# alanqrwang/nwhead

Hardware: AMD Instinct MI355X
Metric: query-predictions/sec (higher is better)
Workload: dtype f32; 1 GPU; K3 predict('full'): B=256 queries/step vs bank N=50000 d=512 C=200, bank sharded 1-way, 26 query batches coalesced per launch; B=256, N_support=50000, d=512, C=200, parallelism=support-shard x1

## Files before the change

### include/nwhead_hip.h

```cpp
#ifndef NWHEAD_HIP_H
#define NWHEAD_HIP_H

#include <stddef.h>
#include <stdint.h>

#ifdef __cplusplus
extern "C" {
#endif

#define NW_ABI_VERSION 2

typedef enum {
    NW_SCORE_EUCLIDEAN = 0,
    NW_SCORE_HYPERSPHERE = 1,
    NW_SCORE_COSINE = 2,
    NW_SCORE_DOT = 3,
    NW_SCORE_CLIP = 4
} nw_score_kind;

typedef enum {
    NW_OK = 0,
    NW_ERR_INVALID_ARG = -1,
    NW_ERR_UNSUPPORTED = -2,
    NW_ERR_WORKSPACE = -3,
    NW_ERR_LAUNCH = -4,
    NW_ERR_NO_DEVICE = -5
} nw_status;

int nw_abi_version(void);
const char *nw_status_string(int status);
int nw_device_check(void);

int nw_scores_f32(const float *q, const float *s, float *scores,
                  int64_t B, int64_t N, int64_t d,
                  int kind, const float *logit_scale_dev, int sup_batched, void *stream);

int nw_row_norm2_f32(const float *x, float *n2, int64_t rows, int64_t d, void *stream);

int nw_split_rows_f16x2(const float *x, float *out_split, float *row_scale, float *row_norm2,
                        int64_t rows, int64_t d, void *stream);

int nw_pack_rows_f16(const float *x, uint16_t *out_rows, float *row_scale, float *row_norm2,
                     int64_t rows, int64_t d, void *stream);

typedef struct nw_fwd_opts {
    uint32_t struct_size;
    int32_t persistent_wgs;
    int32_t force_split;
    int32_t operand_form;
    const void *tables;
    size_t tables_bytes;
    const int64_t *tables_sy;
    int64_t tables_N;
} nw_fwd_opts;

size_t nw_fwd_workspace_bytes(int64_t B, int64_t N, int64_t d, int64_t C);
int nw_fwd_f32(const float *q, const float *s, const int64_t *sy, const float *s_norm2,
               const float *s_split, const float *s_scale,
               float *out, float *scores_out, float *lse_out, float *weights_out,
               void *workspace, size_t workspace_bytes,
               int64_t B, int64_t N, int64_t d, int64_t C,
               int kind, const float *logit_scale_dev,
               int sup_batched, int labels_batched, const nw_fwd_opts *opts, void *stream);

int nw_fwd_partial_f32(const float *q, const float *s, const int64_t *sy, const float *s_norm2,
                       const float *s_split, const float *s_scale,
                       float *m, float *den, float *num,
                       void *workspace, size_t workspace_bytes,
                       int64_t B, int64_t N, int64_t d, int64_t C,
                       int kind, const float *logit_scale_dev, const nw_fwd_opts *opts, void *stream);
int nw_merge_finalize_f32(const float *m, const float *den, const float *num, float *out,
                          int64_t G, int64_t B, int64_t C,
                          int64_t stride_m, int64_t stride_den, int64_t stride_num,
                          const int64_t *class_lo, int64_t C_local, void *stream);

size_t nw_bank_tables_bytes(int64_t N);
int nw_bank_tables_build(const int64_t *sy, int64_t N, int64_t C, void *tables, size_t tables_bytes, void *stream);


size_t nw_bwd_workspace_bytes(int64_t B, int64_t N, int64_t d, int64_t C, int kind, int sup_batched);
int nw_bwd_f32(const float *q, const float *s, const int64_t *sy,
               const float *scores, const float *lse, const float *out, const float *gout,
               float *gq, float *gs, float *glogit_scale,
               void *workspace, size_t workspace_bytes,
               int64_t B, int64_t N, int64_t d, int64_t C,
               int kind, const float *logit_scale_dev,
               int sup_batched, int labels_batched, void *stream);
int nw_bwd_uses_split(int64_t B, int64_t N, int64_t d, int64_t C, int sup_batched);
int nw_bwd_bank_f32(const float *q, const float *s, const float *s_norm2, const float *s_split,
                    const float *s_scale, const int64_t *sy,
                    const float *scores, const float *lse, const float *out, const float *gout,
                    float *gq, float *gs, float *glogit_scale,
                    void *workspace, size_t workspace_bytes,
                    int64_t B, int64_t N, int64_t d, int64_t C,
                    int kind, const float *logit_scale_dev,
                    int sup_batched, int labels_batched, void *stream);


int nw_support_influence_f32(const float *probs, const int64_t *qy, const float *w,
                             const int64_t *sy, float *infl,
                             int64_t B, int64_t N, int64_t C, void *stream);

int nw_aggregate_f32(const float *scores, const int64_t *sy, float *out, float *lse_out, float *weights_out,
                     int64_t B, int64_t N, int64_t C, int labels_batched, void *stream);
int nw_aggregate_bwd_f32(const float *scores, const int64_t *sy, const float *lse, const float *out, const float *gout,
                         float *gscores, int64_t B, int64_t N, int64_t C, int labels_batched, void *stream);

int nw_fwd_influence_f32(const float *q, const float *s, const int64_t *sy, const float *s_norm2,
                         const float *s_split, const float *s_scale, const int64_t *qy,
                         float *out, float *lse_out, float *infl_out,
                         void *workspace, size_t workspace_bytes,
                         int64_t B, int64_t N, int64_t d, int64_t C,
                         int kind, const float *logit_scale_dev, const nw_fwd_opts *opts, void *stream);

int nw_topk_f32(const float *scores, int64_t *idx_out, float *val_out,
                int64_t B, int64_t N, int64_t k, void *stream);

size_t nw_knn_workspace_bytes(int64_t B, int64_t N, int64_t d, int64_t k);
int nw_knn_f32(const float *q, const float *s_split, const float *s_scale, const float *s_norm2,
               int64_t *idx_out, float *val_out, void *workspace, size_t workspace_bytes,
               int64_t B, int64_t N, int64_t d, int64_t k, int kind, const float *logit_scale_dev,
               void *stream);
int nw_scores_use_split(int64_t B, int64_t N, int64_t d);

int nw_scale_shift_relu_f32(const float *x, const float *scale, const float *shift, float *out,
                            int64_t n, int64_t c, int64_t hw, int64_t x_batch_stride, int relu,
                            void *stream);
int nw_scale_shift_relu_avgpool2_f32(const float *x, const float *scale, const float *shift, float *out,
                                     int64_t n, int64_t c, int64_t h, int64_t w, int64_t x_batch_stride,
// ... 160 lines not shown
```

### nwhead_amd/_lib.py

```python
from __future__ import annotations

import ctypes as C
import os

_HERE = os.path.dirname(os.path.abspath(__file__))
LIB_PATH = os.environ.get("NW_HIP_LIB") or os.path.join(_HERE, "csrc", "libnwhead_hip.so")

SCORE_KINDS = {"euclidean": 0, "hypersphere_euclidean": 1, "cosine": 2, "dotproduct": 3, "clip": 4}

_p = C.c_void_p
_i64 = C.c_int64
_int = C.c_int
_sz = C.c_size_t

SIGNATURES = {
    "nw_abi_version": (_int, []),
    "nw_status_string": (C.c_char_p, [_int]),
    "nw_device_check": (_int, []),
    "nw_scores_f32": (_int, [_p, _p, _p, _i64, _i64, _i64, _int, _p, _int, _p]),
    "nw_fwd_workspace_bytes": (_sz, [_i64, _i64, _i64, _i64]),
    "nw_row_norm2_f32": (_int, [_p, _p, _i64, _i64, _p]),
    "nw_split_rows_f16x2": (_int, [_p, _p, _p, _p, _i64, _i64, _p]),
    "nw_pack_rows_f16": (_int, [_p, _p, _p, _p, _i64, _i64, _p]),
    "nw_fwd_f32": (_int, [_p, _p, _p, _p, _p, _p, _p, _p, _p, _p, _p, _sz, _i64, _i64, _i64, _i64, _int, _p, _int, _int, _p, _p]),
    "nw_fwd_partial_f32": (_int, [_p, _p, _p, _p, _p, _p, _p, _p, _p, _p, _sz, _i64, _i64, _i64, _i64, _int, _p, _p, _p]),
    "nw_merge_finalize_f32": (_int, [_p, _p, _p, _p, _i64, _i64, _i64, _i64, _i64, _i64, _p, _i64, _p]),
    "nw_bank_tables_bytes": (_sz, [_i64]),
    "nw_bank_tables_build": (_int, [_p, _i64, _i64, _p, _sz, _p]),
    "nw_bwd_workspace_bytes": (_sz, [_i64, _i64, _i64, _i64, _int, _int]),
    "nw_bwd_f32": (_int, [_p] * 10 + [_p, _sz, _i64, _i64, _i64, _i64, _int, _p, _int, _int, _p]),
    "nw_bwd_uses_split": (_int, [_i64, _i64, _i64, _i64, _int]),
    "nw_bwd_bank_f32": (_int, [_p] * 13 + [_p, _sz, _i64, _i64, _i64, _i64, _int, _p, _int, _int, _p]),
    "nw_support_influence_f32": (_int, [_p, _p, _p, _p, _p, _i64, _i64, _i64, _p]),
    "nw_aggregate_f32": (_int, [_p] * 5 + [_i64, _i64, _i64, _int, _p]),
    "nw_aggregate_bwd_f32": (_int, [_p] * 6 + [_i64, _i64, _i64, _int, _p]),
    "nw_fwd_influence_f32": (_int, [_p] * 11 + [_sz, _i64, _i64, _i64, _i64, _int, _p, _p, _p]),
    "nw_topk_f32": (_int, [_p, _p, _p, _i64, _i64, _i64, _p]),
    "nw_knn_workspace_bytes": (_sz, [_i64, _i64, _i64, _i64]),
    "nw_scores_use_split": (_int, [_i64, _i64, _i64]),
    "nw_knn_f32": (_int, [_p, _p, _p, _p, _p, _p, _p, _sz, _i64, _i64, _i64, _i64, _int, _p, _p]),
    "nw_scale_shift_relu_f32": (_int, [_p, _p, _p, _p, _i64, _i64, _i64, _i64, _int, _p]),
    "nw_bias_act_nhwc_f32": (_int, [_p, _p, _p, _int, _p, _i64, _i64, _p]),
    "nw_scale_shift_relu_avgpool2_f32": (_int, [_p, _p, _p, _p, _i64, _i64, _i64, _i64, _i64, _int, _p]),
    "nw_conv3x3_workgroups": (_i64, [_i64, _i64, _i64, _i64, _i64]),
    "nw_conv3x3_workspace_bytes": (_sz, [_i64, _i64, _i64, _i64, _i64]),
    "nw_conv3x3_f32": (_int, [_p, _i64, _p, _p, _p, _i64, _int, _p, _i64, _p, _sz, _i64, _i64, _i64, _i64, _i64, _p]),
    "nw_conv1x1_workspace_bytes": (_sz, [_i64, _i64, _i64, _i64]),
    "nw_conv1x1_f32": (_int, [_p, _i64, _p, _p, _int, _p, _p, _int, _p, _i64, _p, _sz, _i64, _i64, _i64, _i64, _p]),
    "nw_bn_relu_train_fwd_f32": (_int, [_p] * 10 + [_i64, _i64, _i64, _i64, C.c_float, C.c_float, _int, _p]),
    "nw_bn_relu_train_bwd_f32": (_int, [_p] * 12 + [_i64, _i64, _i64, _i64, _i64, _int, _p]),
    "nw_absmax_f32": (_int, [_p, _i64, _p, _p]),
    "nw_to_nhwc_pad_f32": (_int, [_p, _p, _p, _i64, _i64, _i64, _i64, _i64, _i64, _i64, _p]),
    "nw_conv2d_nhwc_supported": (_int, [_i64] * 9),
    "nw_conv2d_nhwc_f16x2": (_int, [_p, _p, _p, _p, _p, _p, _int, _p, _p] + [_i64] * 11 + [_p, _p]),
    "nw_conv2d_nhwc_moments_groups": (_i64, [_i64] * 9),
    "nw_conv2d_nhwc_bnstat_f16x2": (_int, [_p, _p, _p, _p, _p, _p] + [_i64] * 11 + [_p, _p]),
    "nw_bn_relu_nhwc_train_bwd_from_partials_f32": (_int, [_p, _i64] + [_p] * 6 + [_i64, _p, _p, _p, _p, _i64, _i64, _p, _p, _sz, _i64,
                                                           _i64, _p]),
    "nw_stem7x7s2_relu_maxpool_supported": (_int, [_i64] * 4),
    "nw_stem7x7s2_relu_maxpool_f16x2": (_int, [_p] * 7 + [_i64] * 4 + [_p]),
    "nw_bn_relu_avgpool2x2_nhwc_f32": (_int, [_p, _i64, _p, _p, _i64, _p, _i64, _i64, _i64, _i64, _p]),
    "nw_add_relu_f32": (_int, [_p, _p, _p, _p, _i64, _p]),
    "nw_relu_bwd_f32": (_int, [_p, _p, _p, _p, _i64, _p]),
    "nw_bn_dgrad1x1_workspace_bytes": (_sz, [_i64, _i64]),
    "nw_bn_dgrad1x1_bwd_f16x2": (_int, [_p, _p, _p, _p, _p, _i64, _p, _i64, _p, _p, _i64, _p, _p, _p, _p, _sz, _i64, _i64, _i64, _p]),
    "nw_bn_nhwc_moments_f32": (_int, [_p, _i64, _i64, _i64, C.c_float, _p, _p, _p, _p, _sz, _p]),
    "nw_bn_nhwc_moments_from_partials_f32": (_int, [_p, _i64, _i64, C.c_float, _p, _p, _p, _p]),
    "nw_bn_nhwc_moments_minmax_f32": (_int, [_p, _i64, _i64, _i64, C.c_float, _p, _p, _p, _p, _p, _p, _sz, _p]),
    "nw_bn_nhwc_minmax_workspace_bytes": (_sz, [_i64, _i64]),
    "nw_bn_nhwc_prep_from_partials_f32": (_int, [_p, _i64, _i64, C.c_float, _p, _p, _p, _p, _p, _p, _p, _p, _p, _p, C.c_float, _int,
                                                 _p, _p, _p]),
    "nw_bn_nhwc_prep_window_from_partials_f32": (_int, [_p, _i64, _i64, _i64, _i64, _i64, C.c_float, _p, _p, _p, _p, _p, _p, _p, _p, _p,
                                                        _p, C.c_float, _int, _p, _p, _p]),
    "nw_bn_nhwc_prep_f32": (_int, [_p, _p, _p, _p, _p, _p, _p, _p, _p, _p, C.c_float, _int, _i64, _i64, _p, _p, _p]),
    "nw_conv2d_nhwc_bnrelu_f16x2": (_int, [_p] * 3 + [_i64] + [_p] * 3 + [_int, _p, _p] + [_i64] * 11 + [_p, _p]),
    "nw_bn_relu_nhwc_apply_f32": (_int, [_p, _i64] + [_p] * 8 + [C.c_float, _p, _p, _i64, _i64, _int, _p]),
    "nw_split_conv_weights_f16x2": (_int, [_p, _i64, _i64, _p, _p, _p]),
    "nw_conv2d_nhwc_wgrad_supported": (_int, [_i64] * 9),
    "nw_conv2d_nhwc_wgrad_workspace_bytes": (_sz, [_i64] * 9),
    "nw_conv2d_nhwc_wgrad_f16x2": (_int, [_p, _p, _p, _p, _p, _p, _sz] + [_i64] * 11 + [_p]),
# ... 98 lines not shown
```

### nwhead_amd/csrc/fused.hip

```cpp
#include <mutex>
#include <utility>
#include <vector>
#include "fused_impl.h"
#include <cstring>

namespace nw {

#define NW_EXTERN_FUSED_KIND(K)                                                                          \
    extern template int launch_fused_kind<K>(const float*, const float*, const int64_t*, const float*,   \
                                             const float*,                                               \
                                             const float*, float*, float*, float*, float*, float*,       \
                                             float*, void*, size_t, int, int, int, int, hipStream_t, const CandOut*); \
    extern template int launch_fused_half_kind<K>(const float*, const void*, const int64_t*, const float*, const float*, \
                                                  const float*, float*, float*, float*, float*, float*, void*, size_t,   \
                                                  int, int, int, int, hipStream_t);
NW_EXTERN_FUSED_KIND(NW_SCORE_EUCLIDEAN)
NW_EXTERN_FUSED_KIND(NW_SCORE_HYPERSPHERE)
NW_EXTERN_FUSED_KIND(NW_SCORE_COSINE)
NW_EXTERN_FUSED_KIND(NW_SCORE_DOT)
NW_EXTERN_FUSED_KIND(NW_SCORE_CLIP)
#undef NW_EXTERN_FUSED_KIND

namespace {
struct TileTimer {
// ... 55 lines not shown
}

int device_cu_count() {
    static int n = [] {
        int dev = 0, v = 0;
        if (hipGetDevice(&dev) != hipSuccess) return 256;
        if (hipDeviceGetAttribute(&v, hipDeviceAttributeMultiprocessorCount, dev) != hipSuccess || v <= 0) return 256;
        return v;
    }();
    return n;
}
bool env_flag(const char* name) {
    static const struct { const char* n; int k; } map[] = {
        {"NW_MERGE_PER_QUERY", KNOB_MERGE_PER_QUERY}, {"NW_MERGE_NO_GLOBAL_TABLES", KNOB_MERGE_NO_GLOBAL_TABLES},
        {"NW_PERSISTENT_ANY_RS", KNOB_PERSISTENT_ANY_RS}, {"NW_NO_PERSISTENT", KNOB_NO_PERSISTENT}};
    for (const auto& m : map)
        if (!strcmp(m.n, name)) return knob(m.k) == 1;
    return false;
}

inline size_t al256(size_t x) { return (x + 255) & ~(size_t)255; }

size_t fused_layout(int64_t B, int64_t n_stiles, int BS, char* base, FusedWs* ws, int64_t C) {
    size_t off = 0;
    auto take = [&](size_t bytes) {
        char* p = base ? base + off : nullptr;
        off += al256(bytes);
        return p;
    };
    FusedWs w;
    w.m = reinterpret_cast<float*>(take((size_t)n_stiles * B * 4));
    w.den = reinterpret_cast<float*>(take((size_t)n_stiles * B * 4));
    w.nrun = reinterpret_cast<int*>(take((size_t)n_stiles * 4));
    w.lab = reinterpret_cast<int*>(take((size_t)n_stiles * BS * 4));
    w.num = reinterpret_cast<float*>(take((size_t)n_stiles * BS * B * 4));
    w.runid = reinterpret_cast<int*>(take(((size_t)n_stiles * BS + 64) * 4));
    w.bnd = reinterpret_cast<int*>(take((size_t)n_stiles * 2 * 4));
    w.ctab = reinterpret_cast<int*>(take((size_t)C * (3 + 4) * 4));
    if (ws) *ws = w;
    return off;
}

namespace {

constexpr int MTHREADS = 512, MENT = 4, MTPT = 16;
template <bool PARTIAL, int MQ, int TMODE>
__global__ __launch_bounds__(MTHREADS) void nw_merge_runs_kernel(
    const float* __restrict__ ws_m, const float* __restrict__ ws_den, const int* __restrict__ ws_nrun,
    const int* __restrict__ ws_lab, const float* __restrict__ ws_num, float* __restrict__ out,
    float* __restrict__ lse, float* __restrict__ m_out, float* __restrict__ den_out,
    float* __restrict__ num_out, int B, int C, int n_stiles, int BS, const int* __restrict__ ctab) {
    constexpr bool TABLES = TMODE != 0;
    constexpr bool LTAB = TMODE == 1;
    constexpr int ML = MTHREADS / MQ;
    constexpr int MNS = MQ + 1;
    constexpr int NW = MTHREADS / 64;
    constexpr float LN2 = 0.693147180559945309417f;
    static_assert(MQ <= 32 && (MQ & (MQ - 1)) == 0, "a wave holds whole groups of MQ queries");
    extern __shared__ __attribute__((aligned(16))) char smem[];
    float* red = reinterpret_cast<float*>(smem);
    float* Ms = red + 2 * NW * MQ;
    float* inv_s = Ms + MQ;
    int* lds_tab = reinterpret_cast<int*>(inv_s + MQ);
    int* cnt = TMODE == 2 ? const_cast<int*>(ctab) : lds_tab;
    int* tlo = cnt + C;
    int* thi = tlo + C;
    int* ent = thi + C;
    float* res = reinterpret_cast<float*>(lds_tab + (size_t)C * (3 + MENT));
    const int tid = threadIdx.x, bq = tid & (MQ - 1), sl = tid / MQ, wave = tid >> 6;
    const int b0 = blockIdx.x * MQ;
    const int b = min(b0 + bq, B - 1);

    const bool in_regs = n_stiles <= ML * MTPT;
    float mr[MTPT], dr[MTPT];
    float M = -INFINITY;
    if (in_regs) {
#pragma unroll
        for (int u = 0; u < MTPT; ++u) {
            const int t = sl + u * ML;
            const bool ok = t < n_stiles;
            mr[u] = ok ? ws_m[(size_t)t * B + b] : -INFINITY;
            dr[u] = ok ? ws_den[(size_t)t * B + b] : 0.f;
        }
    }
    int tnr = 0, tl3[3] = {-1, -1, -1};
    const bool one_pass_tables = LTAB && n_stiles <= MTHREADS;
    if (one_pass_tables && tid < n_stiles) {
        tnr = ws_nrun[tid];
        const int* lt = ws_lab + (size_t)tid * BS;
        tl3[0] = lt[0];
        tl3[1] = lt[1];
        tl3[2] = lt[2];
    }
    if (LTAB) {
        for (int c = tid; c < C; c += MTHREADS) {
            cnt[c] = 0;
            tlo[c] = 0x7fffffff;
            thi[c] = -1;
        }
    }
    if (in_regs) {
#pragma unroll
        for (int u = 0; u < MTPT; ++u) M = fmaxf(M, mr[u]);
    } else {
        for (int t = sl; t < n_stiles; t += ML) M = fmaxf(M, ws_m[(size_t)t * B + b]);
    }
#pragma unroll
    for (int o = 32; o >= MQ; o >>= 1) M = fmaxf(M, __shfl_xor(M, o));
    if ((tid & 63) < MQ) red[wave * MQ + bq] = M;
    __syncthreads();
    if (LTAB) {
        auto add_tile = [&](int t, int nr, const int (&l3)[3]) {
            const int* lt = ws_lab + (size_t)t * BS;
            for (int r = 0; r < nr; ++r) {
                const int y = r < 3 ? l3[r] : lt[r];
                if (y < 0) continue;
                atomicMin(&tlo[y], t);
                atomicMax(&thi[y], t);
                const int slot = atomicAdd(&cnt[y], 1);
                if (slot < MENT) ent[y * MENT + slot] = t * BS + r;
            }
// ... 5 lines not shown
                const int* lt = ws_lab + (size_t)t * BS;
                const int l3[3] = {lt[0], lt[1], lt[2]};
                add_tile(t, ws_nrun[t], l3);
            }
        }
    }
    M = red[bq];
#pragma unroll
    for (int k = 1; k < NW; ++k) M = fmaxf(M, red[k * MQ + bq]);
    float den = 0.f;
    if (in_regs) {
#pragma unroll
        for (int u = 0; u < MTPT; ++u) den += dr[u] * __builtin_amdgcn_exp2f(mr[u] - M);
    } else {
        for (int t = sl; t < n_stiles; t += ML)
            den += ws_den[(size_t)t * B + b] * __builtin_amdgcn_exp2f(ws_m[(size_t)t * B + b] - M);
    }
#pragma unroll
    for (int o = 32; o >= MQ; o >>= 1) den += __shfl_xor(den, o);
    if ((tid & 63) < MQ) red[NW * MQ + wave * MQ + bq] = den;
    if (sl == 0) Ms[bq] = M;
    __syncthreads();
    if (LTAB) {
        for (int c = tid; c < C; c += MTHREADS) {
            const int n = cnt[c];
            if (n > 1 && n <= MENT) {
                int e[MENT];
#pragma unroll
                for (int k = 0; k < MENT; ++k) e[k] = k < n ? ent[c * MENT + k] : 0x7fffffff;
#pragma unroll
                for (int i = 1; i < MENT; ++i)
#pragma unroll
                    for (int j = MENT - 1; j >= i; --j)
                        if (e[j] < e[j - 1]) { const int x = e[j]; e[j] = e[j - 1]; e[j - 1] = x; }
#pragma unroll
                for (int k = 0; k < MENT; ++k)
                    if (k < n) ent[c * MENT + k] = e[k];
            }
        }
    }
    den = red[NW * MQ + bq];
#pragma unroll
    for (int k = 1; k < NW; ++k) den += red[NW * MQ + k * MQ + bq];
    if (sl == 0) inv_s[bq] = 1.f / den;
    const int nq = min(MQ, B - b0);
    if (sl == 0 && bq < nq) {
        if (PARTIAL) {
            m_out[b] = M * LN2;
            den_out[b] = den;
        } else if (lse) {
            lse[b] = M * LN2 + logf(den);
        }
    }
    __syncthreads();
    int P = 1;
    while (P < 64 && 2 * P * C * MQ <= MTHREADS) P <<= 1;
    for (int xx = tid; xx < C * MQ * P; xx += MTHREADS) {
        const int x = xx / P, sub = xx - x * P;
        const int c = x / MQ, q = x - c * MQ;
        const int bb = min(b0 + q, B - 1);
        const float Mq = Ms[q];
        float acc = 0.f;
        const int n = TABLES ? cnt[c] : MENT + 1;
        if (n <= MENT) {
            int e[MENT];
            float v[MENT], mt[MENT];
#pragma unroll
            for (int k = 0; k < MENT; ++k) e[k] = ent[c * MENT + (k < n ? k : 0)];
#pragma unroll
            for (int k = 0; k < MENT; ++k) {
                if (k < n) {
                    v[k] = ws_num[(size_t)e[k] * B + bb];
                    mt[k] = ws_m[(size_t)(e[k] / BS) * B + bb];
                }
            }
#pragma unroll
            for (int k = 0; k < MENT; ++k)
                if (k < n) acc += v[k] * __builtin_amdgcn_exp2f(mt[k] - Mq);
        } else {
            const int t0 = TABLES ? tlo[c] : 0, t1 = TABLES ? thi[c] : n_stiles - 1;
            for (int t = t0 + sub; t <= t1; t += P) {
                const int nr = ws_nrun[t];
                const float f = __builtin_amdgcn_exp2f(ws_m[(size_t)t * B + bb] - Mq);
                const int* lt = ws_lab + (size_t)t * BS;
                for (int r = 0; r < nr; ++r)
                    if (lt[r] == c) acc += ws_num[((size_t)t * BS + r) * B + bb] * f;
            }
        }
        if (P > 1) {
            if (n <= MENT && sub != 0) acc = 0.f;
            for (int o = P >> 1; o > 0; o >>= 1) acc += __shfl_xor(acc, o);
            if (sub != 0) continue;
        }
        if (LTAB && MQ > 1) {
            res[c * MNS + q] = acc;
        } else if (q < nq) {
            if (PARTIAL) num_out[(size_t)bb * C + c] = acc;
            else out[(size_t)bb * C + c] = logf(acc * inv_s[q] + NW_LOG_EPS);
        }
    }
    if (!LTAB || MQ == 1) return;
    __syncthreads();
    for (int x = tid; x < nq * C; x += MTHREADS) {
        const int qq = x / C, c = x - qq * C;
        if (PARTIAL) num_out[(size_t)(b0 + qq) * C + c] = res[c * MNS + qq];
        else out[(size_t)(b0 + qq) * C + c] = logf(res[c * MNS + qq] * inv_s[qq] + NW_LOG_EPS);
    }
}

__global__ __launch_bounds__(1024) void nw_class_tables_kernel(const int* __restrict__ ws_nrun, const int* __restrict__ ws_lab,
                                                                int n_stiles, int BS, int C, int* __restrict__ ctab) {
    int* cnt = ctab;
    int* tlo = cnt + C;
    int* thi = tlo + C;
    int* ent = thi + C;
    const int tid = threadIdx.x;
    for (int c = tid; c < C; c += 1024) {
        cnt[c] = 0;
        tlo[c] = 0x7fffffff;
        thi[c] = -1;
    }
    __threadfence();
    __syncthreads();
    for (int t = tid; t < n_stiles; t += 1024) {
        const int nr = ws_nrun[t];
        const int* lt = ws_lab + (size_t)t * BS;
        for (int r = 0; r < nr; ++r) {
            const int y = lt[r];
            if (y < 0) continue;
            atomicMin(&tlo[y], t);
            atomicMax(&thi[y], t);
            const int slot = atomicAdd(&cnt[y], 1);
            if (slot < MENT) ent[y * MENT + slot] = t * BS + r;
        }
    }
    __threadfence();
    __syncthreads();
    for (int c = tid; c < C; c += 1024) {
        const int n = cnt[c];
        if (n > 1 && n <= MENT) {
            int e[MENT];
#pragma unroll
            for (int k = 0; k < MENT; ++k) e[k] = k < n ? ent[c * MENT + k] : 0x7fffffff;
#pragma unroll
            for (int i = 1; i < MENT; ++i)
#pragma unroll
                for (int j = MENT - 1; j >= i; --j)
                    if (e[j] < e[j - 1]) { const int x = e[j]; e[j] = e[j - 1]; e[j - 1] = x; }
#pragma unroll
            for (int k = 0; k < MENT; ++k)
                if (k < n) ent[c * MENT + k] = e[k];
        }
    }
}
// ... 12 lines not shown
        if (t < BS && j < N) y = sy[j];
        lab[u] = ((uint64_t)y < (uint64_t)C) ? (int)y : -1;
    }
    const int prev_last = __shfl_up(lab[2], 1);
    flag[0] = (lane == 0) || (lab[0] != prev_last);
    flag[1] = lab[1] != lab[0];
    flag[2] = lab[2] != lab[1];
    int incl = flag[0] + flag[1] + flag[2];
#pragma unroll
    for (int o = 1; o < 64; o <<= 1) {
        const int v = __shfl_up(incl, o);
        if (lane >= o) incl += v;
    }
    int id = incl - (flag[0] + flag[1] + flag[2]) - 1;
#pragma unroll
    for (int u = 0; u < 3; ++u) {
        const int t = 3 * lane + u;
        id += flag[u];
        if (t < BS) {
            runid[(size_t)s0 + t] = id;
            if (flag[u]) lab_out[(size_t)s0 + id] = lab[u];
            if (flag[u] && (id == 1 || id == 2)) bnd[2 * st + id - 1] = t;
            if (t == BS - 1) nrun[st] = id + 1;
        }
    }
}

int env_rs() {
    const int v = knob(KNOB_TILE_RS);
    return v == KNOB_UNSET ? 0 : v;
}

}

int query_area_of_workspace(void* workspace, size_t workspace_bytes, int64_t B, int64_t N, int64_t d, int64_t C, float** rows,
                            float** scale, float** norm2) {
    const size_t total = nw_fwd_workspace_bytes(B, N, d, C);
    if (!workspace || workspace_bytes < total) return NW_ERR_WORKSPACE;
    const size_t a = al256((size_t)B * (size_t)d * sizeof(float)), b = al256((size_t)B * sizeof(float));
    char* base = static_cast<char*>(workspace) + (total - a - 3 * b);
    *rows = reinterpret_cast<float*>(base);
    *scale = reinterpret_cast<float*>(base + a);
    *norm2 = reinterpret_cast<float*>(base + a + b);
    return NW_OK;
}

int split_queries_into_workspace(const float* q, void* workspace, size_t workspace_bytes, int64_t B, int64_t N, int64_t d,
                                 int64_t C, float** rows, float** scale, float** norm2, hipStream_t st) {
    const int rc = query_area_of_workspace(workspace, workspace_bytes, B, N, d, C, rows, scale, norm2);
    if (rc != NW_OK) return rc;
    return launch_split_rows(q, *rows, *scale, *norm2, B, d, st);
}

int launch_run_tables(const FusedWs& ws, const int64_t* sy, int N, int C, int n_stiles, int BS, hipStream_t st) {
    if (BS > 192) return NW_ERR_UNSUPPORTED;
    hipLaunchKernelGGL(nw_run_tables_kernel, dim3(n_stiles), dim3(64), 0, st, sy, N, C, BS, ws.runid, ws.nrun, ws.lab, ws.bnd);
    NW_CHECK_LAUNCH();
    return NW_OK;
}

constexpr int BANK_BS = 128;

size_t bank_tables_layout(int64_t n_stiles, char* base, FusedWs* ws) {
    size_t off = 0;
    auto take = [&](size_t bytes) {
        char* p = base ? base + off : nullptr;
        off += al256(bytes);
        return p;
    };
    int* nrun = reinterpret_cast<int*>(take((size_t)n_stiles * 4));
    int* lab = reinterpret_cast<int*>(take((size_t)n_stiles * BANK_BS * 4));
    int* runid = reinterpret_cast<int*>(take(((size_t)n_stiles * BANK_BS + 64) * 4));
    int* bnd = reinterpret_cast<int*>(take((size_t)n_stiles * 2 * 4));
    if (ws) {
        ws->nrun = nrun;
        ws->lab = lab;
        ws->runid = runid;
        ws->bnd = bnd;
    }
    return off;
}

bool bank_tables_take(const int64_t* sy, int N, int C, int n_stiles, int BS, FusedWs* ws) {
    (void)C;
    const FwdOpts& o = fwd_opts();
    if (!o.tables || BS != BANK_BS) return false;
    if (o.tables_sy != sy || o.tables_N != (int64_t)N) return false;
    if (o.tables_bytes < bank_tables_layout(n_stiles, nullptr, nullptr)) return false;
    bank_tables_layout(n_stiles, const_cast<char*>(o.tables), ws);
    return true;
}

int launch_merge_runs(const FusedWs& ws, float* out, float* lse, float* m, float* den, float* num,
                      int B, int C, int n_stiles, int BS, hipStream_t st) {
    auto lds_bytes = [&](int mq, bool tables) {
        return ((size_t)2 * (MTHREADS / 64) * mq + 2 * mq + (tables ? (size_t)C * (3 + MENT + mq + 1) : 0)) * sizeof(float);
    };
    const size_t cap = 150 * 1024;
    int mq = 1;
    const int force_mq = knob(KNOB_MERGE_MQ) == KNOB_UNSET ? 0 : knob(KNOB_MERGE_MQ);
    if (force_mq == 1 || force_mq == 16 || force_mq == 32) {
        mq = force_mq;
        if (lds_bytes(mq, true) > cap) mq = 1;
    } else if (B >= 512 && !env_flag("NW_MERGE_PER_QUERY")) {
        mq = n_stiles >= 128 ? 16 : 32;
        if (lds_bytes(mq, true) > cap) mq = 16;
        if (lds_bytes(mq, true) > cap) mq = 1;
    }
    const bool tables = lds_bytes(mq, true) <= cap;
    const size_t lds = lds_bytes(mq, tables);
    const int grid = (B + mq - 1) / mq;
#define NW_MERGE(P_, Q_, T_)                                                                                       \
    hipLaunchKernelGGL((nw_merge_runs_kernel<P_, Q_, T_>), dim3(grid), dim3(MTHREADS), lds, st, ws.m, ws.den, ws.nrun, \
                       ws.lab, ws.num, out, lse, m, den, num, B, C, n_stiles, BS, ws.ctab)
    if (!tables) {
        if (ws.ctab && !env_flag("NW_MERGE_NO_GLOBAL_TABLES")) {
            hipLaunchKernelGGL(nw_class_tables_kernel, dim3(1), dim3(1024), 0, st, ws.nrun, ws.lab, n_stiles, BS, C, ws.ctab);
            if (out) NW_MERGE(false, 1, 2); else NW_MERGE(true, 1, 2);
        } else {
            if (out) NW_MERGE(false, 1, 0); else NW_MERGE(true, 1, 0);
        }
    } else if (mq == 1) {
        if (out) NW_MERGE(false, 1, 1); else NW_MERGE(true, 1, 1);
    } else if (mq == 16) {
        if (out) NW_MERGE(false, 16, 1); else NW_MERGE(true, 16, 1);
    } else {
        if (out) NW_MERGE(false, 32, 1); else NW_MERGE(true, 32, 1);
    }
#undef NW_MERGE
    NW_CHECK_LAUNCH();
    return NW_OK;
}

int pick_rs(int64_t B, int64_t N, int64_t d, bool f16) {
    const int forced = env_rs();
    if (forced == 2 || forced == 4 || forced == 5 || forced == 6 || forced == 8 || forced == 10 || forced == 12)
        return forced;
    const int64_t nq = (B + BQ - 1) / BQ;
    if (forced == 0 && !f16 && d % BK == 0 && nq * ((N + 79) / 80) >= 480) return 5;
    if (forced == 0 && f16 && d % BK == 0 && nq * ((N + 127) / 128) >= 4 * 256) return 8;
    const int cand[] = {2, 4, 6, 8, 10, 12};
    const int ncand = f16 ? 5 : 6;
    double best = 1e30;
    int best_rs = 8;
    for (int ci = 0; ci < ncand; ++ci) {
        const int rs = cand[ci];
        const int64_t ns = (N + 16 * rs - 1) / (16 * rs);
        const int64_t nwg = nq * ns;
        const int64_t rounds = (nwg + 255) / 256;
        double cost = (double)rounds * (rs + 1.5);
        if (nwg >= 384) cost *= 0.85;
        if (cost < best - 1e-9) {
            best = cost;
            best_rs = rs;
        }
    }
    return best_rs;
}

size_t fused_workspace_bytes(int64_t B, int64_t N, int64_t d, int64_t C) {
    size_t need = 0;
    for (int f16 = 0; f16 < 2; ++f16) {
        const int rs = pick_rs(B, N, d, f16 != 0);
        const int64_t n_stiles = (N + 16 * rs - 1) / (16 * rs);
        const size_t n = fused_layout(B, n_stiles, 16 * rs, nullptr, nullptr, C);
        need = n > need ? n : need;
    }
    if (half_form_shape_ok(d)) {
        const size_t n = fused_layout(B, (N + BANK_BS - 1) / BANK_BS, BANK_BS, nullptr, nullptr, C);
        need = n > need ? n : need;
// ... 75 lines not shown
    w.cand.k = (int)k;
    if (out) *out = w;
    return off;
}
}

size_t knn_workspace_bytes(int64_t B, int64_t N, int64_t d, int64_t k) {
    if (!knn_shape_ok(B, N, d, k) || B == 0) return 0;
    if (pick_rs(B, N, d, true) > 10) return 0;
    size_t need = knn_layout(B, N, d, k, nullptr, nullptr);
    const int64_t nq = (B + BQ - 1) / BQ;
    for (int64_t qt = 1; qt <= nq && qt < 1024; ++qt) {
        const int64_t Bq = qt * BQ < B ? qt * BQ : B;
        for (int64_t n = 17; n <= N && qt * ((n + 127) / 128) < 1024; n += 16) {
            const int64_t nn = n > 26 ? n : 26;
            if (nn > N || k > nn) continue;
            const size_t x = knn_layout(Bq, nn, d, k, nullptr, nullptr);
            need = x > need ? x : need;
        }
    }
    return need;
}

int launch_knn(const float* q, const float* s_split, const float* s_scale, const float* s_norm2, int64_t* idx, float* vals,
               void* workspace, size_t workspace_bytes, int64_t B, int64_t N, int64_t d, int64_t k, int kind, const float* ls,
               hipStream_t st) {
    if (!knn_shape_ok(B, N, d, k)) return NW_ERR_UNSUPPORTED;
    if (B == 0) return NW_OK;
    KnnWs w;
    const size_t need = knn_layout(B, N, d, k, static_cast<char*>(workspace), &w);
    if (!workspace || workspace_bytes < need) return NW_ERR_WORKSPACE;
    if (w.n_stiles * w.kcp >= (1ll << 31)) return NW_ERR_UNSUPPORTED;
    int rc;
#define NW_KIND_CASE(K)                                                                                                     \
    case K:                                                                                                                 \
        rc = launch_fused_kind<K>(q, s_split, nullptr, s_norm2, s_scale, ls, nullptr, nullptr, nullptr, nullptr, nullptr,   \
                                  nullptr, nullptr, 0, (int)B, (int)N, (int)d, 1, st, &w.cand);                             \
        break
    switch (kind) {
        NW_KIND_CASE(NW_SCORE_EUCLIDEAN);
        NW_KIND_CASE(NW_SCORE_HYPERSPHERE);
        NW_KIND_CASE(NW_SCORE_COSINE);
        NW_KIND_CASE(NW_SCORE_DOT);
        NW_KIND_CASE(NW_SCORE_CLIP);
        default: return NW_ERR_UNSUPPORTED;
    }
#undef NW_KIND_CASE
    if (rc != NW_OK) return rc;
    return launch_topk_candidates(w.cand.key, w.cand.row, idx, vals, B, w.n_stiles * w.kcp, k, st);
}

}

extern "C" size_t nw_bank_tables_bytes(int64_t N) {
    if (N <= 0 || N > 0x7fffffffLL) return 0;
    return nw::bank_tables_layout((N + nw::BANK_BS - 1) / nw::BANK_BS, nullptr, nullptr);
}

extern "C" int nw_bank_tables_build(const int64_t* sy, int64_t N, int64_t C, void* tables, size_t tables_bytes,
                                    void* stream) {
    using namespace nw;
    if (N < 0 || C < 0 || N > 0x7fffffffLL || C > 0x7fffffffLL) return NW_ERR_INVALID_ARG;
    if (N == 0) return NW_OK;
    if (!sy || !tables || (reinterpret_cast<uintptr_t>(tables) & 15)) return NW_ERR_INVALID_ARG;
    const int64_t n_stiles = (N + BANK_BS - 1) / BANK_BS;
    FusedWs ws;
    if (tables_bytes < bank_tables_layout(n_stiles, static_cast<char*>(tables), &ws)) return NW_ERR_WORKSPACE;
    return launch_run_tables(ws, sy, (int)N, (int)C, (int)n_stiles, BANK_BS, static_cast<hipStream_t>(stream));
}
```

### nwhead_amd/csrc/fused_impl.h

```cpp
#pragma once
#include <type_traits>
#include "tile_core.h"
#include "tile_dma.h"
#include "tile_f16.h"

namespace nw {

constexpr int RUN_CAP = 192;

struct FusedWs {
    float* m;
    float* den;
    int* nrun;
    int* lab;
    float* num;
    int* runid;
    int* bnd;
    int* ctab;
};
size_t fused_layout(int64_t B, int64_t n_stiles, int BS, char* base, FusedWs* ws, int64_t C = 0);
int launch_run_tables(const FusedWs& ws, const int64_t* sy, int N, int C, int n_stiles, int BS, hipStream_t st);
bool bank_tables_take(const int64_t* sy, int N, int C, int n_stiles, int BS, FusedWs* ws);
int launch_merge_runs(const FusedWs& ws, float* out, float* lse, float* m, float* den, float* num,
                      int B, int C, int n_stiles, int BS, hipStream_t st);
int split_queries_into_workspace(const float* q, void* workspace, size_t workspace_bytes, int64_t B, int64_t N, int64_t d,
                                 int64_t C, float** rows, float** scale, float** norm2, hipStream_t st);
int query_area_of_workspace(void* workspace, size_t workspace_bytes, int64_t B, int64_t N, int64_t d, int64_t C, float** rows,
                            float** scale, float** norm2);
struct CandOut {
    unsigned* key;
    int* row;
    int k;
    float *q_rows, *q_scale, *q_norm2;
};
__host__ __device__ inline int cand_slots(int k, int BS) { return ((k < BS ? k : BS) + 3) & ~3; }
int device_cu_count();
bool env_flag(const char* name);
int tile_timer_start(hipStream_t st);
void tile_timer_stop(int slot, hipStream_t st);
int persistent_qgroup();
int persistent_variant();

namespace {

enum { MODE_REG = 0, MODE_DMA = 1, MODE_DMA_SN = 2, MODE_F16 = 3, MODE_F16Q = 4 };
constexpr bool mode_is_f16(int m) { return m == MODE_F16 || m == MODE_F16Q; }
enum { OUT_NONE = 0, OUT_SCORES = 1, OUT_CAND = 2 };

template <int BS>
__device__ __forceinline__ void run_scan_wave(const int (&lab)[3], int lane, int* runid, int* runlab, int* nrun_s) {
    int flag[3];
    if (lane < 2) nrun_s[1 + lane] = BS;
    const int prev_last = __shfl_up(lab[2], 1);
    flag[0] = (lane == 0) || (lab[0] != prev_last);
    flag[1] = lab[1] != lab[0];
    flag[2] = lab[2] != lab[1];
    int incl = flag[0] + flag[1] + flag[2];
#pragma unroll
    for (int o = 1; o < 64; o <<= 1) {
        const int v = __shfl_up(incl, o);
        if (lane >= o) incl += v;
    }
    int id = incl - (flag[0] + flag[1] + flag[2]) - 1;
#pragma unroll
    for (int u = 0; u < 3; ++u) {
        const int t = 3 * lane + u;
        id += flag[u];
        if (t < BS) {
            runid[t] = id;
            if (flag[u] && (id == 1 || id == 2)) nrun_s[id] = t;
            if (flag[u]) runlab[id] = lab[u];
// ... 529 lines not shown
```

### nwhead_amd/ops.py

```python
from __future__ import annotations

import ctypes
import os

import torch
from torch.autograd.function import once_differentiable

from . import _lib
from ._lib import SCORE_KINDS, NWHipError


_raw_stream = getattr(torch._C, "_cuda_getCurrentRawStream", None)


def _stream(t: torch.Tensor):
    if _raw_stream is not None:
        idx = t.device.index
        return _raw_stream(torch.cuda.current_device() if idx is None else idx)
    return torch.cuda.current_stream(t.device).cuda_stream


class _OnDevice:
    __slots__ = ("ctx",)

# ... 187 lines not shown
        if precision not in ("fp32", "fp16"):
            raise ValueError(f"precision must be 'fp32' or 'fp16', got {precision!r}")
        self.precision = precision
        _need_hip(s, labels)
        lib = _lib.load()
        sc = _f32c(s)
        self._src = _sig(s)
        self.label_max = None
        if labels is not None and labels.numel():
            lo, hi = (int(v) for v in torch.aminmax(labels.detach()))
            if lo < 0:
                raise ValueError("support labels must be non-negative class indices (F.one_hot, nw.py:276, raises too)")
            self.label_max = hi
        self.pad, self.rows = 0, None
        half = precision == "fp16" and sc.dim() == 2 and sc.shape[0] > 25
        if half:
            self.pad = max(192, -(-sc.shape[1] // 64) * 64) - sc.shape[1]
            if self.pad:
                sc = self.rows = torch.nn.functional.pad(sc, (0, self.pad))
        elif precision == "fp32" and sc.dim() == 2 and sc.shape[1] % 32 and sc.shape[1] >= 64 and sc.shape[0] > 0:
            self.pad = (-sc.shape[1]) % 32
            sc = self.rows = torch.nn.functional.pad(sc, (0, self.pad))
        self.sorted_rows = self.sorted_labels = None
        if labels is not None and sc.dim() == 2 and labels.dim() == 1 and labels.numel() > 1:
            lab = labels.detach().to(torch.int64)
            if bool((lab[1:] < lab[:-1]).any()):
                perm = torch.argsort(lab, stable=True)
                self.sorted_rows, self.sorted_labels = sc[perm].contiguous(), lab[perm].contiguous()
                self._labels_ref = labels
                sc = self.sorted_rows
        N, d = sc.shape
        self.shape = (N, d)
        self.split = self.scale = None
        self.packed = self.packed_scale = self.packed_norm2 = None
        if half:
            self.packed = torch.empty(N, d, dtype=torch.float16, device=sc.device)
            self.packed_scale = torch.empty(N, dtype=torch.float32, device=sc.device)
            self.packed_norm2 = torch.empty(N, dtype=torch.float32, device=sc.device)
            with torch.cuda.device(sc.device):
                _lib.check(lib.nw_pack_rows_f16(_ptr(sc), _ptr(self.packed), _ptr(self.packed_scale), _ptr(self.packed_norm2),
                                                N, d, _stream(sc)), "nw_pack_rows_f16")
            self.norm2 = row_norm2(sc)
        elif precision == "fp32" and d % 32 == 0 and N > 0:
            self.split = torch.empty_like(sc)
            self.scale = torch.empty(N, dtype=torch.float32, device=sc.device)
            self.norm2 = torch.empty(N, dtype=torch.float32, device=sc.device)
            with torch.cuda.device(sc.device):
                _lib.check(lib.nw_split_rows_f16x2(_ptr(sc), _ptr(self.split), _ptr(self.scale), _ptr(self.norm2),
                                                   N, d, _stream(sc)), "nw_split_rows_f16x2")
        else:
            self.norm2 = row_norm2(sc)
        self.tables = self._tables_src = None
        self.tables_label_max = -1
        self._opts = {}
        if labels is not None and labels.dim() == 1 and (self.split is not None or self.packed is not None):
            self.build_tables(self.sorted_labels if self.sorted_labels is not None else labels)

    def build_tables(self, labels):
        lib = _lib.load()
        lab = labels.detach()
        lab64 = lab if (lab.dtype == torch.int64 and lab.is_contiguous()) else lab.to(torch.int64).contiguous()
        N = self.shape[0]
        if lab64.dim() != 1 or lab64.numel() != N or N == 0 or not lab64.is_cuda:
            return
        lo, hi = (int(v) for v in torch.aminmax(lab64))
        if lo < 0:
            raise ValueError("support labels must be non-negative class indices (F.one_hot, nw.py:276, raises too)")
        self.tables_label_max = hi
        nbytes = lib.nw_bank_tables_bytes(N)
        tables = torch.empty(max(nbytes, 1), dtype=torch.uint8, device=lab64.device)
        with torch.cuda.device(lab64.device):
            _lib.check(lib.nw_bank_tables_build(_ptr(lab64), N, 0x7fffffff, _ptr(tables), nbytes, _stream(lab64)),
                       "nw_bank_tables_build")
        self.tables, self._tables_src, self._opts = tables, _sig(labels), {}

    def call_opts(self, sy, n_classes, persistent_wgs=0, sy_call=None, operand_form=0):
        if self.tables is not None and _sig(sy) == self._tables_src:
            syc = sy if sy_call is None else sy_call
            if self.tables_label_max >= int(n_classes):
                raise ValueError(f"support label {self.tables_label_max} is outside [0, n_classes={int(n_classes)}) "
                                 "(the reference's F.one_hot, nw.py:276, raises)")
            key = (int(persistent_wgs), _lib.force_split(), syc.data_ptr(), syc.numel(), int(operand_form))
            op = self._opts.get(key)
            if op is None:
                if len(self._opts) > 64:
                    self._opts.clear()
                op = self._opts[key] = _lib.fwd_opts(self.tables.data_ptr(), self.tables.numel(), persistent_wgs,
                                                     syc.data_ptr(), syc.numel(), operand_form)
            return C_addr(op)
        return _default_opts(persistent_wgs, operand_form)

    def half_operands(self, d):
        if self.packed is None:
            return None
        if d != self.shape[1]:
            raise ValueError(f"queries of width {d} against an fp16 bank of (padded) width {self.shape[1]}")
        return self.packed_norm2, self.packed, self.packed_scale

    def matches(self, s):
        return _sig(s) == self._src


def _resolve_sorted_bank(s, sy, cache, per_position_outputs=False):
    if cache is None or cache.sorted_rows is None:
        return s, sy, cache
    same = sy is cache._labels_ref or (sy.data_ptr() == cache._labels_ref.data_ptr() and sy.shape == cache._labels_ref.shape)
    if per_position_outputs or not same:
        return s, sy, None
    return cache.sorted_rows, cache.sorted_labels, cache


def _apply_bank_padding(q, s, cache):
    if cache is None or not cache.pad:
        return q, s
    q = torch.nn.functional.pad(q, (0, cache.pad))
    if s.shape[-1] != cache.shape[1]:
        s = cache.rows
    return q, s


class _NoCtx:
    needs_input_grad = (False, False, False, False)

    @staticmethod
    def mark_non_differentiable(*a):
        pass

# ... 1370 lines not shown
```

### nwhead_amd/sharded.py

```python
from __future__ import annotations

import torch
import torch.distributed as dist

from . import ops


def shard_bounds(n_rows: int, world: int, rank: int):
    base, extra = divmod(n_rows, world)
    lo = rank * base + min(rank, extra)
    return lo, lo + base + (1 if rank < extra else 0)


def _coalesce(chunk):
    first = chunk[0]
    if first.is_contiguous() and first.dim() == 2:
        base = first.untyped_storage().data_ptr()
        step = first.numel() * first.element_size()
        if all(c.dtype == first.dtype and c.shape == first.shape and c.is_contiguous() and
               c.untyped_storage().data_ptr() == base and c.data_ptr() == first.data_ptr() + k * step
               for k, c in enumerate(chunk)):
            return first.as_strided((len(chunk) * first.shape[0], first.shape[1]), (first.shape[1], 1))
    return torch.cat(chunk, dim=0)


class ShardedBank:
    def __init__(self, feat_shard, y_shard, n_classes, kind="euclidean", logit_scale=None, group=None,
                 partial_fn=None, merge_fn=None, persistent_wgs=None, precision="fp32"):
        self.feat = feat_shard.detach().to(torch.float32).contiguous()
        self.y = y_shard.detach().to(torch.int64).contiguous()
        self.C = int(n_classes)
        self.kind, self.logit_scale, self.group = kind, logit_scale, group
        self.world = dist.get_world_size(group) if dist.is_initialized() else 1
        self._partial = partial_fn or self._hip_partial
        self._merge = merge_fn or self._hip_merge
        self._ws = None
        if persistent_wgs is None:
            persistent_wgs = 0
            if self.world > 1 and self.feat.is_cuda:
                cus = torch.cuda.get_device_properties(self.feat.device).multi_processor_count
                persistent_wgs = max(8, (cus - 8) // 8 * 8)
        self.persistent_wgs = int(persistent_wgs)
        self.class_lo, self.CL, self.y_local = None, self.C, self.y
        if self.world > 1:
            lo = int(self.y.min()) if self.y.numel() else 0
            hi = int(self.y.max()) if self.y.numel() else -1
            box = torch.tensor([lo, hi], dtype=torch.int64, device=self.feat.device)
            allb = torch.empty(self.world, 2, dtype=torch.int64, device=self.feat.device)
            dist.all_gather_into_tensor(allb.view(-1), box, group=group)
            width = int((allb[:, 1] - allb[:, 0] + 1).clamp_min(1).max())
            if width < self.C:
                self.CL = width
                self.class_lo = allb[:, 0].clamp(0, max(self.C - 1, 0)).contiguous()
                self.y_local = (self.y - lo).contiguous()
        self.cache = ops.SplitBank(self.feat, precision=precision) if (partial_fn is None and self.feat.is_cuda) else None
        self.norm2 = self.cache.norm2 if self.cache is not None else None
        if self.cache is not None and (self.cache.split is not None or self.cache.packed is not None):
            self.cache.build_tables(self.y_local)

    def _hip_partial(self, packed_row, q):
        N, d = self.feat.shape
        if self.cache is not None and self.cache.pad:
            d = self.cache.shape[1]
        B = q.shape[0]
        need = ops._lib.load().nw_fwd_workspace_bytes(B, N, d, self.CL)
        if self._ws is None or self._ws.numel() < need:
            self._ws = torch.empty(max(need, 1), dtype=torch.uint8, device=q.device)
        ops.nw_partials_into(packed_row, q, self.feat, self.y_local, self.CL, self.kind, self.logit_scale,
                             ws=self._ws, cache=self.cache, persistent_wgs=self.persistent_wgs)

    def _hip_merge(self, gathered_rows, B):
        return ops.nw_merge(gathered_rows, B, self.C, class_lo=self.class_lo, c_local=self.CL)

    def row_len(self, B):
        return 2 * B + B * self.CL

    def predict(self, q):
        return self.predict_stream([q], bucket=1)[0]

    def predict_stream(self, batches, bucket=8):
        if not batches:
            return []
        d = batches[0].shape[-1]
        for k, qb in enumerate(batches):
            if qb.dim() != 2 or qb.shape[1] != d:
                raise ValueError(f"predict_stream: batch {k} has shape {tuple(qb.shape)}, expected (B, {d})")
        dev, G = self.feat.device, self.world
        outs, pending = [], None
        ring = {}

        def split(out, sizes):
            pos = 0
            for n in sizes:
                outs.append(out[pos:pos + n])
                pos += n

        def finish(p):
            work, gathered, sizes = p
            if work is not None:
                work.wait()
            split(self._merge(gathered, sum(sizes)), sizes)

        for n_bucket, i0 in enumerate(range(0, len(batches), bucket)):
            chunk = batches[i0:i0 + bucket]
            sizes = [int(c.shape[0]) for c in chunk]
            Bq = sum(sizes)
            L = self.row_len(Bq)
            key = (n_bucket % 3, Bq)
            if key not in ring:
                ring[key] = (torch.empty(L, dtype=torch.float32, device=dev),
                             torch.empty(G, L, dtype=torch.float32, device=dev))
# ... 18 lines not shown
```

Baseline: 7.993 million query-predictions/s.

## Prebuild per-class merge tables with bank tables and shrink merge LDS

Class tables (counts and run bounds per class) are now built once alongside the bank's run tables, when the label set is known, and stored after them in the bank table buffer. The merge kernel can then read these prepared global tables (mode 2) instead of rebuilding them in LDS on every launch. It also drops the LDS table region, which shrinks per-block LDS and removes one barrier. The price is extra bank-table memory and a C-dependent buffer size, and the layout match now hinges on the table byte count equalling the layout computed for C.

```diff
diff --git a/include/nwhead_hip.h b/include/nwhead_hip.h
--- a/include/nwhead_hip.h
+++ b/include/nwhead_hip.h
@@ -74,7 +74,11 @@
                           int64_t stride_m, int64_t stride_den, int64_t stride_num,
                           const int64_t *class_lo, int64_t C_local, void *stream);
 
-size_t nw_bank_tables_bytes(int64_t N);
+#ifdef __cplusplus
+size_t nw_bank_tables_bytes(int64_t N, int64_t C = 0);
+#else
+size_t nw_bank_tables_bytes(int64_t N, int64_t C);
+#endif
 int nw_bank_tables_build(const int64_t *sy, int64_t N, int64_t C, void *tables, size_t tables_bytes, void *stream);
 
 
diff --git a/nwhead_amd/_lib.py b/nwhead_amd/_lib.py
--- a/nwhead_amd/_lib.py
+++ b/nwhead_amd/_lib.py
@@ -25,7 +25,7 @@
     "nw_fwd_f32": (_int, [_p, _p, _p, _p, _p, _p, _p, _p, _p, _p, _p, _sz, _i64, _i64, _i64, _i64, _int, _p, _int, _int, _p, _p]),
     "nw_fwd_partial_f32": (_int, [_p, _p, _p, _p, _p, _p, _p, _p, _p, _p, _sz, _i64, _i64, _i64, _i64, _int, _p, _p, _p]),
     "nw_merge_finalize_f32": (_int, [_p, _p, _p, _p, _i64, _i64, _i64, _i64, _i64, _i64, _p, _i64, _p]),
-    "nw_bank_tables_bytes": (_sz, [_i64]),
+    "nw_bank_tables_bytes": (_sz, [_i64, _i64]),
     "nw_bank_tables_build": (_int, [_p, _i64, _i64, _p, _sz, _p]),
     "nw_bwd_workspace_bytes": (_sz, [_i64, _i64, _i64, _i64, _int, _int]),
     "nw_bwd_f32": (_int, [_p] * 10 + [_p, _sz, _i64, _i64, _i64, _i64, _int, _p, _int, _int, _p]),
diff --git a/nwhead_amd/csrc/fused.hip b/nwhead_amd/csrc/fused.hip
--- a/nwhead_amd/csrc/fused.hip
+++ b/nwhead_amd/csrc/fused.hip
@@ -131,6 +131,8 @@
     float* __restrict__ num_out, int B, int C, int n_stiles, int BS, const int* __restrict__ ctab) {
     constexpr bool TABLES = TMODE != 0;
     constexpr bool LTAB = TMODE == 1;
+    constexpr bool STAGE = MQ > 1;
+    static_assert(TMODE != 0 || MQ == 1, "the LDS of mode 0 has no room for res");
     constexpr int ML = MTHREADS / MQ;
     constexpr int MNS = MQ + 1;
     constexpr int NW = MTHREADS / 64;
@@ -145,7 +147,7 @@
     int* tlo = cnt + C;
     int* thi = tlo + C;
     int* ent = thi + C;
-    float* res = reinterpret_cast<float*>(lds_tab + (size_t)C * (3 + MENT));
+    float* res = reinterpret_cast<float*>(lds_tab + (LTAB ? (size_t)C * (3 + MENT) : 0));
     const int tid = threadIdx.x, bq = tid & (MQ - 1), sl = tid / MQ, wave = tid >> 6;
     const int b0 = blockIdx.x * MQ;
     const int b = min(b0 + bq, B - 1);
@@ -257,7 +259,7 @@
             lse[b] = M * LN2 + logf(den);
         }
     }
-    __syncthreads();
+    if (LTAB || !STAGE) __syncthreads();
     int P = 1;
     while (P < 64 && 2 * P * C * MQ <= MTHREADS) P <<= 1;
     for (int xx = tid; xx < C * MQ * P; xx += MTHREADS) {
@@ -297,14 +299,14 @@
             for (int o = P >> 1; o > 0; o >>= 1) acc += __shfl_xor(acc, o);
             if (sub != 0) continue;
         }
-        if (LTAB && MQ > 1) {
+        if (STAGE) {
             res[c * MNS + q] = acc;
         } else if (q < nq) {
             if (PARTIAL) num_out[(size_t)bb * C + c] = acc;
             else out[(size_t)bb * C + c] = logf(acc * inv_s[q] + NW_LOG_EPS);
         }
     }
-    if (!LTAB || MQ == 1) return;
+    if (!STAGE) return;
     __syncthreads();
     for (int x = tid; x < nq * C; x += MTHREADS) {
         const int qq = x / C, c = x - qq * C;
@@ -423,6 +425,12 @@
     return launch_split_rows(q, *rows, *scale, *norm2, B, d, st);
 }
 
+int launch_class_tables(const FusedWs& ws, int n_stiles, int BS, int C, hipStream_t st) {
+    hipLaunchKernelGGL(nw_class_tables_kernel, dim3(1), dim3(1024), 0, st, ws.nrun, ws.lab, n_stiles, BS, C, ws.ctab);
+    NW_CHECK_LAUNCH();
+    return NW_OK;
+}
+
 int launch_run_tables(const FusedWs& ws, const int64_t* sy, int N, int C, int n_stiles, int BS, hipStream_t st) {
     if (BS > 192) return NW_ERR_UNSUPPORTED;
     hipLaunchKernelGGL(nw_run_tables_kernel, dim3(n_stiles), dim3(64), 0, st, sy, N, C, BS, ws.runid, ws.nrun, ws.lab, ws.bnd);
@@ -432,7 +440,7 @@
 
 constexpr int BANK_BS = 128;
 
-size_t bank_tables_layout(int64_t n_stiles, char* base, FusedWs* ws) {
+size_t bank_tables_layout(int64_t n_stiles, int64_t C, char* base, FusedWs* ws) {
     size_t off = 0;
     auto take = [&](size_t bytes) {
         char* p = base ? base + off : nullptr;
@@ -443,30 +451,38 @@
     int* lab = reinterpret_cast<int*>(take((size_t)n_stiles * BANK_BS * 4));
     int* runid = reinterpret_cast<int*>(take(((size_t)n_stiles * BANK_BS + 64) * 4));
     int* bnd = reinterpret_cast<int*>(take((size_t)n_stiles * 2 * 4));
+    int* ctab = reinterpret_cast<int*>(base ? base + off : nullptr);
+    off += (size_t)C * (3 + MENT) * 4;
     if (ws) {
         ws->nrun = nrun;
         ws->lab = lab;
         ws->runid = runid;
         ws->bnd = bnd;
+        if (C > 0) {
+            ws->ctab = ctab;
+            ws->ctab_built = true;
+        }
     }
     return off;
 }
 
 bool bank_tables_take(const int64_t* sy, int N, int C, int n_stiles, int BS, FusedWs* ws) {
-    (void)C;
     const FwdOpts& o = fwd_opts();
     if (!o.tables || BS != BANK_BS) return false;
     if (o.tables_sy != sy || o.tables_N != (int64_t)N) return false;
-    if (o.tables_bytes < bank_tables_layout(n_stiles, nullptr, nullptr)) return false;
-    bank_tables_layout(n_stiles, const_cast<char*>(o.tables), ws);
+    if (o.tables_bytes < bank_tables_layout(n_stiles, 0, nullptr, nullptr)) return false;
+    const bool ctab = C > 0 && o.tables_bytes == bank_tables_layout(n_stiles, C, nullptr, nullptr);
+    bank_tables_layout(n_stiles, ctab ? C : 0, const_cast<char*>(o.tables), ws);
     return true;
 }
 
 int launch_merge_runs(const FusedWs& ws, float* out, float* lse, float* m, float* den, float* num,
                       int B, int C, int n_stiles, int BS, hipStream_t st) {
-    auto lds_bytes = [&](int mq, bool tables) {
-        return ((size_t)2 * (MTHREADS / 64) * mq + 2 * mq + (tables ? (size_t)C * (3 + MENT + mq + 1) : 0)) * sizeof(float);
+    auto lds_bytes_of = [&](int mq, bool ltab, bool stage) {
+        return ((size_t)2 * (MTHREADS / 64) * mq + 2 * mq + (ltab ? (size_t)C * (3 + MENT) : 0) +
+                (stage ? (size_t)C * (mq + 1) : 0)) * sizeof(float);
     };
+    auto lds_bytes = [&](int mq, bool tables) { return lds_bytes_of(mq, tables, tables); };
     const size_t cap = 150 * 1024;
     int mq = 1;
     const int force_mq = knob(KNOB_MERGE_MQ) == KNOB_UNSET ? 0 : knob(KNOB_MERGE_MQ);
@@ -479,14 +495,20 @@
         if (lds_bytes(mq, true) > cap) mq = 1;
     }
     const bool tables = lds_bytes(mq, true) <= cap;
-    const size_t lds = lds_bytes(mq, tables);
+    const bool prepared = ws.ctab_built && ws.ctab && tables;
+    const size_t lds = prepared ? lds_bytes_of(mq, false, mq > 1) : lds_bytes(mq, tables);
     const int grid = (B + mq - 1) / mq;
 #define NW_MERGE(P_, Q_, T_)                                                                                       \
     hipLaunchKernelGGL((nw_merge_runs_kernel<P_, Q_, T_>), dim3(grid), dim3(MTHREADS), lds, st, ws.m, ws.den, ws.nrun, \
                        ws.lab, ws.num, out, lse, m, den, num, B, C, n_stiles, BS, ws.ctab)
-    if (!tables) {
+    if (prepared) {
+        if (mq == 1) { if (out) NW_MERGE(false, 1, 2); else NW_MERGE(true, 1, 2); }
+        else if (mq == 16) { if (out) NW_MERGE(false, 16, 2); else NW_MERGE(true, 16, 2); }
+        else { if (out) NW_MERGE(false, 32, 2); else NW_MERGE(true, 32, 2); }
+    } else if (!tables) {
         if (ws.ctab && !env_flag("NW_MERGE_NO_GLOBAL_TABLES")) {
-            hipLaunchKernelGGL(nw_class_tables_kernel, dim3(1), dim3(1024), 0, st, ws.nrun, ws.lab, n_stiles, BS, C, ws.ctab);
+            if (!ws.ctab_built)
+                hipLaunchKernelGGL(nw_class_tables_kernel, dim3(1), dim3(1024), 0, st, ws.nrun, ws.lab, n_stiles, BS, C, ws.ctab);
             if (out) NW_MERGE(false, 1, 2); else NW_MERGE(true, 1, 2);
         } else {
             if (out) NW_MERGE(false, 1, 0); else NW_MERGE(true, 1, 0);
@@ -668,9 +690,9 @@
 
 }
 
-extern "C" size_t nw_bank_tables_bytes(int64_t N) {
-    if (N <= 0 || N > 0x7fffffffLL) return 0;
-    return nw::bank_tables_layout((N + nw::BANK_BS - 1) / nw::BANK_BS, nullptr, nullptr);
+extern "C" size_t nw_bank_tables_bytes(int64_t N, int64_t C) {
+    if (N <= 0 || N > 0x7fffffffLL || C < 0 || C > 0x7fffffffLL) return 0;
+    return nw::bank_tables_layout((N + nw::BANK_BS - 1) / nw::BANK_BS, C, nullptr, nullptr);
 }
 
 extern "C" int nw_bank_tables_build(const int64_t* sy, int64_t N, int64_t C, void* tables, size_t tables_bytes,
@@ -681,6 +703,8 @@
     if (!sy || !tables || (reinterpret_cast<uintptr_t>(tables) & 15)) return NW_ERR_INVALID_ARG;
     const int64_t n_stiles = (N + BANK_BS - 1) / BANK_BS;
     FusedWs ws;
-    if (tables_bytes < bank_tables_layout(n_stiles, static_cast<char*>(tables), &ws)) return NW_ERR_WORKSPACE;
-    return launch_run_tables(ws, sy, (int)N, (int)C, (int)n_stiles, BANK_BS, static_cast<hipStream_t>(stream));
-}
+    if (tables_bytes < bank_tables_layout(n_stiles, C, static_cast<char*>(tables), &ws)) return NW_ERR_WORKSPACE;
+    const int rc = launch_run_tables(ws, sy, (int)N, (int)C, (int)n_stiles, BANK_BS, static_cast<hipStream_t>(stream));
+    if (rc != NW_OK || C == 0) return rc;
+    return launch_class_tables(ws, (int)n_stiles, BANK_BS, (int)C, static_cast<hipStream_t>(stream));
+}
diff --git a/nwhead_amd/csrc/fused_impl.h b/nwhead_amd/csrc/fused_impl.h
--- a/nwhead_amd/csrc/fused_impl.h
+++ b/nwhead_amd/csrc/fused_impl.h
@@ -16,7 +16,8 @@
     float* num;
     int* runid;
     int* bnd;
-    int* ctab;
+    int* ctab = nullptr;
+    bool ctab_built = false;
 };
 size_t fused_layout(int64_t B, int64_t n_stiles, int BS, char* base, FusedWs* ws, int64_t C = 0);
 int launch_run_tables(const FusedWs& ws, const int64_t* sy, int N, int C, int n_stiles, int BS, hipStream_t st);
diff --git a/nwhead_amd/ops.py b/nwhead_amd/ops.py
--- a/nwhead_amd/ops.py
+++ b/nwhead_amd/ops.py
@@ -263,11 +263,12 @@
             self.norm2 = row_norm2(sc)
         self.tables = self._tables_src = None
         self.tables_label_max = -1
+        self.tables_classes = 0
         self._opts = {}
         if labels is not None and labels.dim() == 1 and (self.split is not None or self.packed is not None):
             self.build_tables(self.sorted_labels if self.sorted_labels is not None else labels)
 
-    def build_tables(self, labels):
+    def build_tables(self, labels, n_classes=None):
         lib = _lib.load()
         lab = labels.detach()
         lab64 = lab if (lab.dtype == torch.int64 and lab.is_contiguous()) else lab.to(torch.int64).contiguous()
@@ -278,12 +279,14 @@
         if lo < 0:
             raise ValueError("support labels must be non-negative class indices (F.one_hot, nw.py:276, raises too)")
         self.tables_label_max = hi
-        nbytes = lib.nw_bank_tables_bytes(N)
+        C = max(hi + 1, int(n_classes) if n_classes is not None else 0)
+        nbytes = lib.nw_bank_tables_bytes(N, C)
         tables = torch.empty(max(nbytes, 1), dtype=torch.uint8, device=lab64.device)
         with torch.cuda.device(lab64.device):
-            _lib.check(lib.nw_bank_tables_build(_ptr(lab64), N, 0x7fffffff, _ptr(tables), nbytes, _stream(lab64)),
+            _lib.check(lib.nw_bank_tables_build(_ptr(lab64), N, C, _ptr(tables), nbytes, _stream(lab64)),
                        "nw_bank_tables_build")
         self.tables, self._tables_src, self._opts = tables, _sig(labels), {}
+        self.tables_classes = C
 
     def call_opts(self, sy, n_classes, persistent_wgs=0, sy_call=None, operand_form=0):
         if self.tables is not None and _sig(sy) == self._tables_src:
diff --git a/nwhead_amd/sharded.py b/nwhead_amd/sharded.py
--- a/nwhead_amd/sharded.py
+++ b/nwhead_amd/sharded.py
@@ -56,7 +56,7 @@
         self.cache = ops.SplitBank(self.feat, precision=precision) if (partial_fn is None and self.feat.is_cuda) else None
         self.norm2 = self.cache.norm2 if self.cache is not None else None
         if self.cache is not None and (self.cache.split is not None or self.cache.packed is not None):
-            self.cache.build_tables(self.y_local)
+            self.cache.build_tables(self.y_local, self.CL)
 
     def _hip_partial(self, packed_row, q):
         N, d = self.feat.shape
```

Measured after the change: 7.952 million query-predictions/s. No clear change (-0.5%).
